# LiangZhaoPKUImperial/LinearSFM

Hardware: AMD Instinct MI355X
Metric: hierarchical linear map-joining solve wall-clock, NC3500-like stereo (all transforms + joins) (lower is better)
Workload: dtype f64

## Files before the change

### linearsfm_amd/csrc/lsfm_small.hip

```cpp
#include "lsfm_device.hpp"
#include "lsfm_internal.hpp"
#include "lsfm_solve.hpp"

namespace lsfm {

#define SM_PASS 16
#define SM_K (3 * SM_PASS)
#define SM_KS (SM_K + 1)
#define SM_THREADS 256
#define SM_CHUNK 256
#define SM_SUPER 64
#define SM_WROWS 1024

typedef double sm_v4d __attribute__((ext_vector_type(4)));

struct SmallArgs {
	int nseg;
	const int *pose_off, *feat_off, *u_off;
	const unsigned char* seg_active;
	const double* U; const int *Ui, *Uj;
	const double* W; const int *photo, *fptr;
	const double* V;
	const double *ea, *eb, *x0;
	const unsigned char* fixed;
	double *x_pose, *x_feat;
	RunStatsDev* run;
	int* status;
	double* max_rel;
	int dbg;
};

template <int NTR>
struct SmallShared {
	static constexpr int R = 16 * NTR;
	double S[R * (R + 1)];
	double P[R * SM_KS];
	double d0[R];
	double E[R], x[R], r[R], v[R], dinv[R];
	double ly[SM_SUPER * 9];
	double wst[SM_WROWS * 3];
	int sph[SM_WROWS / 6 + 1];
	int fpc[2][SM_CHUNK + 1];
	unsigned char fx[R];
	int bad;
	int strips[4];
};

template <int NTR>
#ifndef LSFM_SMALL_OCC
#define LSFM_SMALL_OCC 2
#endif
__global__ void __launch_bounds__(SM_THREADS, NTR >= 6 ? 1 : (NTR <= 2 ? LSFM_SMALL_OCC : 2))
k_small_solve(SmallArgs a)
{
	constexpr int R = 16 * NTR, LD = R + 1;
	constexpr int NTILE = NTR * (NTR + 1) / 2, NW = SM_THREADS / 64, T = (NTILE + NW - 1) / NW;
	extern __shared__ double sm_raw[];
	SmallShared<NTR>& sh = *reinterpret_cast<SmallShared<NTR>*>(sm_raw);
	const int g = blockIdx.x, tid = threadIdx.x, lane = tid & 63, wave = __builtin_amdgcn_readfirstlane(tid >> 6);
	const int p0 = a.pose_off[g], m = a.pose_off[g + 1] - p0, n = 6 * m;
	const int f0 = a.feat_off[g], f1 = a.feat_off[g + 1];
	if (a.seg_active && !a.seg_active[g])
	{
		for (int i = tid; i < n; i += SM_THREADS) a.x_pose[(size_t)p0 * 6 + i] = a.x0 ? a.x0[(size_t)p0 * 6 + i] : 0.0;
		return;
	}
	for (int i = tid; i < R * LD; i += SM_THREADS) sh.S[i] = 0.0;
	for (int i = tid; i < R; i += SM_THREADS)
	{
		sh.E[i] = i < n ? a.ea[(size_t)p0 * 6 + i] : 0.0;
		sh.fx[i] = (i >= n || (a.fixed && a.fixed[(size_t)p0 * 6 + i])) ? 1 : 0;
	}
	if (tid == 0) sh.bad = 0;
	__syncthreads();
	{
		const int u0 = a.u_off[g], u1 = a.u_off[g + 1];
		for (int q = tid; q < (u1 - u0) * 36; q += SM_THREADS)
		{
			const int i = u0 + q / 36, e = q % 36, r = e / 6, c = e % 6;
			const int pa = a.Ui[i] - p0, pb = a.Uj[i] - p0;
			const double v = a.U[(size_t)i * 36 + e];
			lds_add_f64(&sh.S[(6 * pa + r) * LD + 6 * pb + c], v);
			if (pa != pb) lds_add_f64(&sh.S[(6 * pb + c) * LD + 6 * pa + r], v);
		}
	}
	int ti[T], tj[T];
	sm_v4d acc[T];
#pragma unroll
	for (int t = 0; t < T; t++)
	{
		const int q = wave + NW * t;
		int i = 0, j = 0;
		if (q < NTILE)
		{
			while ((j + 1) * (j + 2) / 2 <= q) j++;
			i = q - j * (j + 1) / 2;
		}
		ti[t] = q < NTILE ? i : -1; tj[t] = j;
		acc[t] = (sm_v4d){ 0.0, 0.0, 0.0, 0.0 };
	}
	constexpr int NE = (NTR + NW - 1) / NW;
	double eacc[NE];
#pragma unroll
	for (int i = 0; i < NE; i++) eacc[i] = 0.0;
	const int lbase = (lane & 15) * SM_KS + (lane >> 4);
	constexpr int PF = SM_WROWS / SM_THREADS;
	constexpr int MCAP = R / 6;
	double pw[PF][3];
	int pk[PF];
	double pv[9], pe[3];
	int qbn = 0, c0 = f0, cb = 1;
	auto prefetch = [&](int q0) {
		const int nf = min(SM_SUPER, f1 - q0);
		if (q0 - c0 >= SM_CHUNK || q0 == f0)
		{
			c0 = q0; cb ^= 1;
			for (int i = tid; i <= min(SM_CHUNK, f1 - c0); i += SM_THREADS) sh.fpc[cb][i] = a.fptr[c0 + i];
			__syncthreads();
		}
		qbn = sh.fpc[cb][q0 - c0];
		const int rw = (sh.fpc[cb][q0 - c0 + nf] - qbn) * 6;
		if (tid < nf)
		{
			ld<9>(pv, a.V + (size_t)(q0 + tid) * 9);
			ld<3>(pe, a.eb + (size_t)(q0 + tid) * 3);
		}
		const double* wb = a.W + (size_t)qbn * 18;
#pragma unroll
		for (int i = 0; i < PF; i++)
		{
			const int w = tid + SM_THREADS * i;
			if (w < rw) { pw[i][0] = wb[3 * (size_t)w]; pw[i][1] = wb[3 * (size_t)w + 1]; pw[i][2] = wb[3 * (size_t)w + 2]; pk[i] = a.photo[qbn + w / 6]; }
		}
	};
	for (int i = tid; i < R * SM_KS; i += SM_THREADS) sh.P[i] = 0.0;
	if (f0 < f1) prefetch(f0);
	for (int s0 = f0; s0 < f1; s0 += SM_SUPER)
	{
		const int nfs = min(SM_SUPER, f1 - s0);
		const int qbs = qbn, cs = c0, bs = cb;
		const int rws = (sh.fpc[bs][s0 - cs + nfs] - qbs) * 6;
		__syncthreads();
#pragma unroll
		for (int i = 0; i < PF; i++)
		{
			const int w = tid + SM_THREADS * i;
			if (w < rws)
			{
				sh.wst[3 * w] = pw[i][0]; sh.wst[3 * w + 1] = pw[i][1]; sh.wst[3 * w + 2] = pw[i][2];
				if (w % 6 == 0) sh.sph[w / 6] = pk[i] - p0;
			}
		}
		if (tid < 4) sh.strips[tid] = 0;
		if (tid < SM_SUPER)
		{
			double l[9];
#pragma unroll
			for (int i = 0; i < 9; i++) l[i] = 0.0;
			if (tid < nfs && !(a.dbg & 1))
			{
				double o[9];
				inv3_sym(pv, o);
				const double d0 = o[0];
				l[0] = sqrt(d0); l[1] = o[3] / l[0]; l[3] = o[6] / l[0];
				const double d1 = o[4] - l[1] * l[1];
				l[2] = sqrt(d1); l[4] = (o[7] - l[3] * l[1]) / l[2];
				const double d2 = o[8] - l[3] * l[3] - l[4] * l[4];
				l[5] = sqrt(d2);
				l[6] = l[0] * pe[0] + l[1] * pe[1] + l[3] * pe[2];
				l[7] = l[2] * pe[1] + l[4] * pe[2];
				l[8] = l[5] * pe[2];
				if (!(d0 > 0.0) || !(d1 > 0.0) || !(d2 > 0.0)) sh.bad = 1;
			}
			st<9>(&sh.ly[tid * 9], l);
		}
		__syncthreads();
		if (s0 + SM_SUPER < f1) prefetch(s0 + SM_SUPER);
		for (int sub = 0; sub * SM_PASS < nfs; sub++)
		{
			const int q0 = s0 + sub * SM_PASS, nf = min(SM_PASS, f1 - q0);
			{
				const int lp = tid >> 4, fl = tid & 15;
				bool found = false;
				if (lp < MCAP && !(a.dbg & 2))
				{
					double c18[18];
#pragma unroll
					for (int i = 0; i < 18; i++) c18[i] = 0.0;
					if (fl < nf && lp < m)
					{
						const int j0 = sh.fpc[bs][q0 - cs + fl], j1 = sh.fpc[bs][q0 - cs + fl + 1];
						const double* l = &sh.ly[(sub * SM_PASS + fl) * 9];
						const double l0 = l[0], l1 = l[1], l2 = l[2], l3 = l[3], l4 = l[4], l5 = l[5];
						for (int j = j0; j < j1; j++)
						{
							const int e = j - qbs;
							const int ph = 6 * e < SM_WROWS ? sh.sph[e] : a.photo[j] - p0;
							if (ph != lp) continue;
							found = true;
#pragma unroll
							for (int r = 0; r < 6; r++)
							{
								double w0, w1, w2;
								if (6 * e + 5 < SM_WROWS) { w0 = sh.wst[3 * (6 * e + r)]; w1 = sh.wst[3 * (6 * e + r) + 1]; w2 = sh.wst[3 * (6 * e + r) + 2]; }
								else { const double* wg = a.W + (size_t)j * 18 + 3 * r; w0 = wg[0]; w1 = wg[1]; w2 = wg[2]; }
								c18[3 * r] += w0 * l0 + w1 * l1 + w2 * l3;
								c18[3 * r + 1] += w1 * l2 + w2 * l4;
								c18[3 * r + 2] += w2 * l5;
							}
						}
					}
#pragma unroll
					for (int r = 0; r < 6; r++)
					{
						double* d = &sh.P[(6 * lp + r) * SM_KS + 3 * fl];
						d[0] = c18[3 * r]; d[1] = c18[3 * r + 1]; d[2] = c18[3 * r + 2];
					}
				}
				const int b0 = (6 * lp) >> 4, b1 = (6 * lp + 5) >> 4;
#pragma unroll
				for (int sidx = 0; sidx < NTR; sidx++)
					if (__ballot(found && (b0 == sidx || b1 == sidx)) != 0ull && lane == 0) atomicOr(&sh.strips[sub], 1 << sidx);
			}
			__syncthreads();
			const int smask = sh.strips[sub];
			{
				const int kq = lane >> 4;
#pragma unroll
				for (int si = 0; si < NE; si++)
				{
					const int strip = wave + NW * si;
					if (strip < NTR && ((smask >> strip) & 1) && !(a.dbg & 4))
					{
						const double* pr = &sh.P[(16 * strip + (lane & 15)) * SM_KS + 12 * kq];
						const double* yq = &sh.ly[sub * SM_PASS * 9 + kq * 36 + 6];
						double e0 = 0.0, e1 = 0.0;
#pragma unroll
						for (int k = 0; k < 12; k += 2)
						{
							e0 = fma(pr[k], yq[(k / 3) * 9 + k % 3], e0);
							e1 = fma(pr[k + 1], yq[((k + 1) / 3) * 9 + (k + 1) % 3], e1);
						}
						double sum = e0 + e1;
						sum += __shfl_xor(sum, 16, 64);
						sum += __shfl_xor(sum, 32, 64);
						eacc[si] -= sum;
					}
				}
			}
			bool on[T];
#pragma unroll
			for (int t = 0; t < T; t++) on[t] = ti[t] >= 0 && (((smask >> ti[t]) & (smask >> tj[t]) & 1) != 0) && !(a.dbg & 8);
#pragma unroll 2
			for (int ks = 0; ks < SM_K / 4; ks++)
			{
#pragma unroll
				for (int t = 0; t < T; t++)
				{
					if (!on[t]) continue;
					const double av = sh.P[16 * ti[t] * SM_KS + lbase + 4 * ks], bv = sh.P[16 * tj[t] * SM_KS + lbase + 4 * ks];
					acc[t] = __builtin_amdgcn_mfma_f64_16x16x4f64(av, bv, acc[t], 0, 0, 0);
				}
			}
			__syncthreads();
		}
	}
	__syncthreads();
#pragma unroll
	for (int t = 0; t < T; t++)
	{
		if (ti[t] < 0) continue;
		const int C = 16 * tj[t] + (lane & 15);
#pragma unroll
		for (int e = 0; e < 4; e++)
		{
			const int Rr = 16 * ti[t] + (lane >> 4) + 4 * e;
			const double v = acc[t][e];
			sh.S[Rr * LD + C] -= v;
			if (ti[t] != tj[t]) sh.S[C * LD + Rr] -= v;
		}
	}
	if (lane < 16)
#pragma unroll
		for (int si = 0; si < NE; si++)
		{
			const int strip = wave + NW * si;
			if (strip < NTR) sh.E[16 * strip + lane] += eacc[si];
		}
	__syncthreads();
	for (int q = tid; q < R * R; q += SM_THREADS)
	{
		const int i = q / R, j = q - i * R;
		if (sh.fx[i] || sh.fx[j]) sh.S[i * LD + j] = i == j ? 1.0 : 0.0;
	}
	for (int i = tid; i < R; i += SM_THREADS) if (sh.fx[i]) sh.E[i] = 0.0;
	__syncthreads();
	for (int i = tid; i < R; i += SM_THREADS) sh.d0[i] = sh.S[i * LD + i];
	__syncthreads();
	int pivot_bad = -1;
	for (int j = 0; j < ((a.dbg & 16) ? 0 : n); j++)
	{
		const double d = sh.S[j * LD + j];
		if (!(d > 0.0) || !(d < 1e300)) { pivot_bad = j; break; }
		const double piv = sqrt(d), ip = 1.0 / piv;
		__syncthreads();
		for (int i = j + tid; i < n; i += SM_THREADS) sh.S[i * LD + j] = i == j ? piv : sh.S[i * LD + j] * ip;
		__syncthreads();
		{
			const int ty = tid >> 4, tx = tid & 15;
			for (int i = j + 1 + ty; i < n; i += 16)
			{
				const double lij = sh.S[i * LD + j];
				for (int k = j + 1 + tx; k <= i; k += 16) sh.S[i * LD + k] = fma(-lij, sh.S[k * LD + j], sh.S[i * LD + k]);
			}
		}
		__syncthreads();
	}
	if (pivot_bad >= 0)
	{
		if (tid == 0) { atomicCAS(&a.status[1], 0, 1 + g); if (a.run && !a.run->chol_err) a.run->chol_err = 1 + p0 + pivot_bad / 6; }
		return;
	}
	for (int i = tid; i < n; i += SM_THREADS) sh.dinv[i] = 1.0 / sh.S[i * LD + i];
	__syncthreads();
	auto solve = [&](const double* rhs, double* out) {
		for (int i = tid; i < R; i += SM_THREADS) sh.v[i] = i < n ? rhs[i] : 0.0;
		__syncthreads();
		if (wave == 0)
		{
			for (int j = 0; j < n; j++)
			{
				const double vj = sh.v[j] * sh.dinv[j];
				__builtin_amdgcn_wave_barrier();
				if (lane == 0) sh.v[j] = vj;
				for (int i = j + 1 + lane; i < n; i += 64) sh.v[i] = fma(-sh.S[i * LD + j], vj, sh.v[i]);
				__builtin_amdgcn_wave_barrier();
			}
			for (int j = n - 1; j >= 0; j--)
			{
				const double vj = sh.v[j] * sh.dinv[j];
				__builtin_amdgcn_wave_barrier();
				if (lane == 0) sh.v[j] = vj;
				for (int i = lane; i < j; i += 64) sh.v[i] = fma(-sh.S[j * LD + i], vj, sh.v[i]);
				__builtin_amdgcn_wave_barrier();
			}
		}
		__syncthreads();
		for (int i = tid; i < R; i += SM_THREADS) out[i] = sh.v[i];
		__syncthreads();
	};
	auto residual = [&](const double* xx) {
		for (int i = tid; i < n; i += SM_THREADS)
		{
			double s = sh.E[i] - sh.d0[i] * xx[i];
			for (int j = 0; j < n; j++)
				if (j != i) s = fma(-(i < j ? sh.S[i * LD + j] : sh.S[j * LD + i]), xx[j], s);
			sh.r[i] = s;
		}
		__syncthreads();
	};
	if (!(a.dbg & 16))
	{
	solve(sh.E, sh.x);
	residual(sh.x);
	solve(sh.r, sh.v);
	for (int i = tid; i < n; i += SM_THREADS) sh.x[i] += sh.v[i];
	__syncthreads();
	residual(sh.x);
	}
	if (tid == 0)
	{
		double rr = 0.0, ee = 0.0;
		for (int i = 0; i < n; i++) { rr += sh.r[i] * sh.r[i]; ee += sh.E[i] * sh.E[i]; }
		const double rel = ee > 0.0 ? sqrt(rr / ee) : 0.0;
		if (!(rel < 1e-8) || sh.bad)
		{
			atomicAdd(&a.status[0], 1);
			if (a.run) atomicAdd(&a.run->not_converged, 1);
		}
		const unsigned long long bits = (unsigned long long)__double_as_longlong(rel == rel ? rel : 1e300);
		atomicMax(reinterpret_cast<unsigned long long*>(a.max_rel), bits);
		if (a.run) atomicMax(reinterpret_cast<unsigned long long*>(&a.run->max_rel_residual), bits);
	}
	for (int i = tid; i < n; i += SM_THREADS) a.x_pose[(size_t)p0 * 6 + i] = sh.fx[i] ? 0.0 : sh.x[i];
	for (int f = f0 + tid; f < ((a.dbg & 32) ? f0 : f1); f += SM_THREADS)
	{
		double V[9], iv[9];
		ld<9>(V, a.V + (size_t)f * 9);
		inv3_sym(V, iv);
		double d[3] = { a.eb[(size_t)f * 3], a.eb[(size_t)f * 3 + 1], a.eb[(size_t)f * 3 + 2] };
		double s3[3] = { 0.0, 0.0, 0.0 };
		for (int j = a.fptr[f]; j < a.fptr[f + 1]; j++)
		{
			double w[18];
			ld<18>(w, a.W + (size_t)j * 18);
			const double* xp = &sh.x[6 * (a.photo[j] - p0)];
#pragma unroll
			for (int c = 0; c < 3; c++)
			{
				double sacc = 0.0;
#pragma unroll
				for (int r = 0; r < 6; r++) sacc = fma(w[3 * r + c], sh.fx[6 * (a.photo[j] - p0) + r] ? 0.0 : xp[r], sacc);
				s3[c] += sacc;
			}
		}
		d[0] -= s3[0]; d[1] -= s3[1]; d[2] -= s3[2];
		for (int r = 0; r < 3; r++) a.x_feat[(size_t)f * 3 + r] = iv[3 * r] * d[0] + iv[3 * r + 1] * d[1] + iv[3 * r + 2] * d[2];
	}
}

static int small_solve_strips(int most_poses, int cap)
{
	if (most_poses > cap) return 0;
	if (most_poses <= 2) return 1;
	if (most_poses <= 5) return 2;
	if (most_poses <= 8) return 3;
	if (most_poses <= 16) return 6;
	return 0;
}
int small_level_strips(const lsfm_context* ctx, int most_rows)
{
	return (ctx->small_max > 0 && !ctx->comm && !ctx->pcg.mixed) ? small_solve_strips(most_rows, ctx->small_max) : 0;
}
void small_level_offsets(lsfm_context* ctx, const DevBatch& out, SolveIO& io)
{
	if (!small_level_strips(ctx, io.seg_rows)) return;
	const int G = io.nseg;
	int* d_uo = ctx->scratch.alloc<int>(G + 1);
	h2d(ctx, d_uo, out.u_off.data(), sizeof(int) * (size_t)(G + 1));
	io.d_pose_off = out.d_pose_off; io.d_feat_off = out.d_feat_off; io.d_u_off = d_uo;
}

template <int NTR>
static void launch_small(hipStream_t s, const SmallArgs& a)
{
	const size_t lds = sizeof(SmallShared<NTR>);
	static const bool set = []() {
		(void)hipFuncSetAttribute(reinterpret_cast<const void*>(&k_small_solve<NTR>), hipFuncAttributeMaxDynamicSharedMemorySize, (int)sizeof(SmallShared<NTR>));
		return true;
	}();
	(void)set;
	hipLaunchKernelGGL(k_small_solve<NTR>, dim3(a.nseg), dim3(SM_THREADS), lds, s, a);
}

void small_solve_launch(lsfm_context* ctx, const SolveIO& io, int strips, int* status, double* max_rel)
{
	SmallArgs a;
	a.nseg = io.nseg; a.pose_off = io.d_pose_off; a.feat_off = io.d_feat_off; a.u_off = io.d_u_off; a.seg_active = io.d_seg_active;
	a.U = io.U; a.Ui = io.Ui; a.Uj = io.Uj; a.W = io.W; a.photo = io.photo; a.fptr = io.fptr; a.V = io.V;
	a.ea = io.ea; a.eb = io.eb; a.x0 = io.x0; a.fixed = io.d_fixed; a.x_pose = io.x_pose; a.x_feat = io.x_feat;
	a.run = (ctx->in_tree_run && ctx->d_run) ? ctx->d_run : nullptr;
	a.status = status; a.max_rel = max_rel;
	a.dbg = getenv("LSFM_SMALL_DEBUG") ? atoi(getenv("LSFM_SMALL_DEBUG")) : 0;
	if (!io.nseg) return;
	switch (strips)
	{
	case 1: launch_small<1>(ctx->stream, a); break;
	case 2: launch_small<2>(ctx->stream, a); break;
	case 3: launch_small<3>(ctx->stream, a); break;
	default: launch_small<6>(ctx->stream, a); break;
	}
	LSFM_CHECK_HIP(hipGetLastError());
}

}
```

Baseline: 31.18.

## Give each wave its own feature panel in small Schur kernels to drop block barriers

For the one- and two-tile variants of the small-segment Schur solve, each wave now owns a private P panel and its own slice of the feature super-block. It accumulates all tiles itself and synchronises only at wavefront level instead of with block-wide __syncthreads. Per-wave results are merged into S and E serially, one wave per turn. Photo matching in staging now builds a 32-entry bitmask and iterates its set bits. This is meant to remove block-barrier stalls and idle waves when there are few tiles, at the cost of more LDS for panels and a serialized reduction.

```diff
diff --git a/linearsfm_amd/csrc/lsfm_small.hip b/linearsfm_amd/csrc/lsfm_small.hip
--- a/linearsfm_amd/csrc/lsfm_small.hip
+++ b/linearsfm_amd/csrc/lsfm_small.hip
@@ -5,8 +5,6 @@
 namespace lsfm {
 
 #define SM_PASS 16
-#define SM_K (3 * SM_PASS)
-#define SM_KS (SM_K + 1)
 #define SM_THREADS 256
 #define SM_CHUNK 256
 #define SM_SUPER 64
@@ -31,10 +29,18 @@
 };
 
 template <int NTR>
+struct SmallScheme {
+	static constexpr int WP = NTR == 1 ? 16 : (NTR == 2 ? 8 : 0);
+	static constexpr int PASS = WP ? WP : SM_PASS;
+	static constexpr int KS = 3 * PASS + 1;
+	static constexpr int NPANEL = WP ? SM_THREADS / 64 : 1;
+};
+
+template <int NTR>
 struct SmallShared {
 	static constexpr int R = 16 * NTR;
 	double S[R * (R + 1)];
-	double P[R * SM_KS];
+	double P[SmallScheme<NTR>::NPANEL * R * SmallScheme<NTR>::KS];
 	double d0[R];
 	double E[R], x[R], r[R], v[R], dinv[R];
 	double ly[SM_SUPER * 9];
@@ -45,6 +51,86 @@
 	int bad;
 	int strips[4];
 };
+static_assert(sizeof(SmallShared<1>) <= 80 * 1024 && sizeof(SmallShared<2>) <= 80 * 1024, "k_small_solve<1>, <2>: two work-groups a CU");
+
+template <int KS>
+__device__ __forceinline__ bool sm_stage_cell(const SmallArgs& a, const double* wst, const int* sph, const double* l, bool live, int j0, int j1,
+                                              int qbs, int p0, int lp, double* d)
+{
+	bool found = false;
+	double c18[18];
+#pragma unroll
+	for (int i = 0; i < 18; i++) c18[i] = 0.0;
+	if (live)
+	{
+		const double l0 = l[0], l1 = l[1], l2 = l[2], l3 = l[3], l4 = l[4], l5 = l[5];
+		for (int jb = j0; jb < j1; jb += 32)
+		{
+			unsigned mk = 0;
+			const int je = min(j1, jb + 32);
+#pragma unroll 4
+			for (int j = jb; j < je; j++)
+				mk |= ((6 * (j - qbs) < SM_WROWS ? sph[j - qbs] : a.photo[j] - p0) == lp ? 1u : 0u) << (j - jb);
+			for (; mk; mk &= mk - 1)
+			{
+				const int j = jb + __builtin_ctz(mk);
+				const int e = j - qbs;
+				found = true;
+#pragma unroll
+				for (int r = 0; r < 6; r++)
+				{
+					double w0, w1, w2;
+					if (6 * e + 5 < SM_WROWS) { w0 = wst[3 * (6 * e + r)]; w1 = wst[3 * (6 * e + r) + 1]; w2 = wst[3 * (6 * e + r) + 2]; }
+					else { const double* wg = a.W + (size_t)j * 18 + 3 * r; w0 = wg[0]; w1 = wg[1]; w2 = wg[2]; }
+					c18[3 * r] += w0 * l0 + w1 * l1 + w2 * l3;
+					c18[3 * r + 1] += w1 * l2 + w2 * l4;
+					c18[3 * r + 2] += w2 * l5;
+				}
+			}
+		}
+	}
+#pragma unroll
+	for (int r = 0; r < 6; r++)
+	{
+		d[r * KS] = c18[3 * r]; d[r * KS + 1] = c18[3 * r + 1]; d[r * KS + 2] = c18[3 * r + 2];
+	}
+	return found;
+}
+
+template <int KS>
+__device__ __forceinline__ double sm_strip_py(const double* prow, const double* ly, int kq)
+{
+	constexpr int KQ = (KS - 1) / 4;
+	const double* pr = prow + KQ * kq;
+	const double* yq = ly + kq * (KQ / 3) * 9 + 6;
+	double e0 = 0.0, e1 = 0.0;
+#pragma unroll
+	for (int k = 0; k < KQ; k += 2)
+	{
+		e0 = fma(pr[k], yq[(k / 3) * 9 + k % 3], e0);
+		if (k + 1 < KQ) e1 = fma(pr[k + 1], yq[((k + 1) / 3) * 9 + (k + 1) % 3], e1);
+	}
+	double sum = e0 + e1;
+	sum += __shfl_xor(sum, 16, 64);
+	sum += __shfl_xor(sum, 32, 64);
+	return sum;
+}
+
+template <int KS, int NT, int UNROLL>
+__device__ __forceinline__ void sm_tiles_ppt(const double* pl, const int (&ti)[NT], const int (&tj)[NT], const bool (&on)[NT], sm_v4d (&acc)[NT])
+{
+#pragma unroll UNROLL
+	for (int ks = 0; ks < (KS - 1) / 4; ks++)
+	{
+#pragma unroll
+		for (int t = 0; t < NT; t++)
+		{
+			if (!on[t]) continue;
+			const double av = pl[16 * ti[t] * KS + 4 * ks], bv = pl[16 * tj[t] * KS + 4 * ks];
+			acc[t] = __builtin_amdgcn_mfma_f64_16x16x4f64(av, bv, acc[t], 0, 0, 0);
+		}
+	}
+}
 
 template <int NTR>
 #ifndef LSFM_SMALL_OCC
@@ -54,7 +140,8 @@
 k_small_solve(SmallArgs a)
 {
 	constexpr int R = 16 * NTR, LD = R + 1;
-	constexpr int NTILE = NTR * (NTR + 1) / 2, NW = SM_THREADS / 64, T = (NTILE + NW - 1) / NW;
+	constexpr int WP = SmallScheme<NTR>::WP, PASS = SmallScheme<NTR>::PASS, KS = SmallScheme<NTR>::KS;
+	constexpr int NTILE = NTR * (NTR + 1) / 2, NW = SM_THREADS / 64, T = WP ? NTILE : (NTILE + NW - 1) / NW;
 	extern __shared__ double sm_raw[];
 	SmallShared<NTR>& sh = *reinterpret_cast<SmallShared<NTR>*>(sm_raw);
 	const int g = blockIdx.x, tid = threadIdx.x, lane = tid & 63, wave = __builtin_amdgcn_readfirstlane(tid >> 6);
@@ -89,7 +176,7 @@
 #pragma unroll
 	for (int t = 0; t < T; t++)
 	{
-		const int q = wave + NW * t;
+		const int q = WP ? t : wave + NW * t;
 		int i = 0, j = 0;
 		if (q < NTILE)
 		{
@@ -99,11 +186,11 @@
 		ti[t] = q < NTILE ? i : -1; tj[t] = j;
 		acc[t] = (sm_v4d){ 0.0, 0.0, 0.0, 0.0 };
 	}
-	constexpr int NE = (NTR + NW - 1) / NW;
+	constexpr int NE = WP ? NTR : (NTR + NW - 1) / NW;
 	double eacc[NE];
 #pragma unroll
 	for (int i = 0; i < NE; i++) eacc[i] = 0.0;
-	const int lbase = (lane & 15) * SM_KS + (lane >> 4);
+	const int lbase = (lane & 15) * KS + (lane >> 4);
 	constexpr int PF = SM_WROWS / SM_THREADS;
 	constexpr int MCAP = R / 6;
 	double pw[PF][3];
@@ -133,7 +220,7 @@
 			if (w < rw) { pw[i][0] = wb[3 * (size_t)w]; pw[i][1] = wb[3 * (size_t)w + 1]; pw[i][2] = wb[3 * (size_t)w + 2]; pk[i] = a.photo[qbn + w / 6]; }
 		}
 	};
-	for (int i = tid; i < R * SM_KS; i += SM_THREADS) sh.P[i] = 0.0;
+	for (int i = tid; i < SmallScheme<NTR>::NPANEL * R * KS; i += SM_THREADS) sh.P[i] = 0.0;
 	if (f0 < f1) prefetch(f0);
 	for (int s0 = f0; s0 < f1; s0 += SM_SUPER)
 	{
@@ -151,7 +238,7 @@
 				if (w % 6 == 0) sh.sph[w / 6] = pk[i] - p0;
 			}
 		}
-		if (tid < 4) sh.strips[tid] = 0;
+		if (!WP && tid < 4) sh.strips[tid] = 0;
 		if (tid < SM_SUPER)
 		{
 			double l[9];
@@ -176,118 +263,80 @@
 		}
 		__syncthreads();
 		if (s0 + SM_SUPER < f1) prefetch(s0 + SM_SUPER);
-		for (int sub = 0; sub * SM_PASS < nfs; sub++)
-		{
-			const int q0 = s0 + sub * SM_PASS, nf = min(SM_PASS, f1 - q0);
-			{
-				const int lp = tid >> 4, fl = tid & 15;
+		double* const P = WP ? sh.P + wave * (R * KS) : sh.P;
+		const int id = WP ? lane : tid;
+		constexpr int NL = WP ? 64 : SM_THREADS;
+		auto meet = [&]() {
+			if constexpr (WP != 0) { __builtin_amdgcn_fence(__ATOMIC_ACQ_REL, "wavefront"); __builtin_amdgcn_wave_barrier(); }
+			else __syncthreads();
+		};
+		const int lf_begin = WP ? SM_PASS * wave : 0, lf_end = min(nfs, WP ? SM_PASS * wave + SM_PASS : SM_SUPER);
+		for (int lf0 = lf_begin; lf0 < lf_end; lf0 += PASS)
+		{
+			const int q0 = s0 + lf0, nf = min(PASS, f1 - q0);
+			unsigned seen = 0;
+#pragma unroll
+			for (int c0l = 0; c0l < MCAP * PASS; c0l += NL)
+			{
+				const int c = c0l + id, lp = c / PASS, fl = c % PASS;
 				bool found = false;
 				if (lp < MCAP && !(a.dbg & 2))
 				{
-					double c18[18];
-#pragma unroll
-					for (int i = 0; i < 18; i++) c18[i] = 0.0;
-					if (fl < nf && lp < m)
-					{
-						const int j0 = sh.fpc[bs][q0 - cs + fl], j1 = sh.fpc[bs][q0 - cs + fl + 1];
-						const double* l = &sh.ly[(sub * SM_PASS + fl) * 9];
-						const double l0 = l[0], l1 = l[1], l2 = l[2], l3 = l[3], l4 = l[4], l5 = l[5];
-						for (int j = j0; j < j1; j++)
-						{
-							const int e = j - qbs;
-							const int ph = 6 * e < SM_WROWS ? sh.sph[e] : a.photo[j] - p0;
-							if (ph != lp) continue;
-							found = true;
-#pragma unroll
-							for (int r = 0; r < 6; r++)
-							{
-								double w0, w1, w2;
-								if (6 * e + 5 < SM_WROWS) { w0 = sh.wst[3 * (6 * e + r)]; w1 = sh.wst[3 * (6 * e + r) + 1]; w2 = sh.wst[3 * (6 * e + r) + 2]; }
-								else { const double* wg = a.W + (size_t)j * 18 + 3 * r; w0 = wg[0]; w1 = wg[1]; w2 = wg[2]; }
-								c18[3 * r] += w0 * l0 + w1 * l1 + w2 * l3;
-								c18[3 * r + 1] += w1 * l2 + w2 * l4;
-								c18[3 * r + 2] += w2 * l5;
-							}
-						}
-					}
-#pragma unroll
-					for (int r = 0; r < 6; r++)
-					{
-						double* d = &sh.P[(6 * lp + r) * SM_KS + 3 * fl];
-						d[0] = c18[3 * r]; d[1] = c18[3 * r + 1]; d[2] = c18[3 * r + 2];
-					}
+					const bool live = fl < nf && lp < m;
+					const int j0 = live ? sh.fpc[bs][q0 - cs + fl] : 0, j1 = live ? sh.fpc[bs][q0 - cs + fl + 1] : 0;
+					found = sm_stage_cell<KS>(a, sh.wst, sh.sph, &sh.ly[(lf0 + fl) * 9], live, j0, j1, qbs, p0, lp, &P[6 * lp * KS + 3 * fl]);
 				}
 				const int b0 = (6 * lp) >> 4, b1 = (6 * lp + 5) >> 4;
 #pragma unroll
 				for (int sidx = 0; sidx < NTR; sidx++)
-					if (__ballot(found && (b0 == sidx || b1 == sidx)) != 0ull && lane == 0) atomicOr(&sh.strips[sub], 1 << sidx);
-			}
-			__syncthreads();
-			const int smask = sh.strips[sub];
-			{
-				const int kq = lane >> 4;
+					if (__ballot(found && (b0 == sidx || b1 == sidx)) != 0ull) seen |= 1u << sidx;
+			}
+			if (!WP && lane == 0 && seen) atomicOr(&sh.strips[lf0 / SM_PASS], (int)seen);
+			meet();
+			const int smask = WP ? (int)seen : sh.strips[lf0 / SM_PASS];
+#pragma unroll
+			for (int si = 0; si < NE; si++)
+			{
+				const int strip = WP ? si : wave + NW * si;
+				if (strip < NTR && ((smask >> strip) & 1) && !(a.dbg & 4))
+					eacc[si] -= sm_strip_py<KS>(&P[(16 * strip + (lane & 15)) * KS], &sh.ly[lf0 * 9], lane >> 4);
+			}
+			bool on[T];
+#pragma unroll
+			for (int t = 0; t < T; t++) on[t] = ti[t] >= 0 && (((smask >> ti[t]) & (smask >> tj[t]) & 1) != 0) && !(a.dbg & 8);
+			sm_tiles_ppt<KS, T, (WP ? (KS - 1) / 4 : 2)>(P + lbase, ti, tj, on, acc);
+			meet();
+		}
+	}
+	__syncthreads();
+	for (int turn = 0; turn < (WP ? NW : 1); turn++)
+	{
+		if (!WP || wave == turn)
+		{
+#pragma unroll
+			for (int t = 0; t < T; t++)
+			{
+				if (ti[t] < 0) continue;
+				const int C = 16 * tj[t] + (lane & 15);
+#pragma unroll
+				for (int e = 0; e < 4; e++)
+				{
+					const int Rr = 16 * ti[t] + (lane >> 4) + 4 * e;
+					const double v = acc[t][e];
+					sh.S[Rr * LD + C] -= v;
+					if (ti[t] != tj[t]) sh.S[C * LD + Rr] -= v;
+				}
+			}
+			if (lane < 16)
 #pragma unroll
 				for (int si = 0; si < NE; si++)
 				{
-					const int strip = wave + NW * si;
-					if (strip < NTR && ((smask >> strip) & 1) && !(a.dbg & 4))
-					{
-						const double* pr = &sh.P[(16 * strip + (lane & 15)) * SM_KS + 12 * kq];
-						const double* yq = &sh.ly[sub * SM_PASS * 9 + kq * 36 + 6];
-						double e0 = 0.0, e1 = 0.0;
-#pragma unroll
-						for (int k = 0; k < 12; k += 2)
-						{
-							e0 = fma(pr[k], yq[(k / 3) * 9 + k % 3], e0);
-							e1 = fma(pr[k + 1], yq[((k + 1) / 3) * 9 + (k + 1) % 3], e1);
-						}
-						double sum = e0 + e1;
-						sum += __shfl_xor(sum, 16, 64);
-						sum += __shfl_xor(sum, 32, 64);
-						eacc[si] -= sum;
-					}
+					const int strip = WP ? si : wave + NW * si;
+					if (strip < NTR) sh.E[16 * strip + lane] += eacc[si];
 				}
-			}
-			bool on[T];
-#pragma unroll
-			for (int t = 0; t < T; t++) on[t] = ti[t] >= 0 && (((smask >> ti[t]) & (smask >> tj[t]) & 1) != 0) && !(a.dbg & 8);
-#pragma unroll 2
-			for (int ks = 0; ks < SM_K / 4; ks++)
-			{
-#pragma unroll
-				for (int t = 0; t < T; t++)
-				{
-					if (!on[t]) continue;
-					const double av = sh.P[16 * ti[t] * SM_KS + lbase + 4 * ks], bv = sh.P[16 * tj[t] * SM_KS + lbase + 4 * ks];
-					acc[t] = __builtin_amdgcn_mfma_f64_16x16x4f64(av, bv, acc[t], 0, 0, 0);
-				}
-			}
-			__syncthreads();
-		}
-	}
-	__syncthreads();
-#pragma unroll
-	for (int t = 0; t < T; t++)
-	{
-		if (ti[t] < 0) continue;
-		const int C = 16 * tj[t] + (lane & 15);
-#pragma unroll
-		for (int e = 0; e < 4; e++)
-		{
-			const int Rr = 16 * ti[t] + (lane >> 4) + 4 * e;
-			const double v = acc[t][e];
-			sh.S[Rr * LD + C] -= v;
-			if (ti[t] != tj[t]) sh.S[C * LD + Rr] -= v;
-		}
-	}
-	if (lane < 16)
-#pragma unroll
-		for (int si = 0; si < NE; si++)
-		{
-			const int strip = wave + NW * si;
-			if (strip < NTR) sh.E[16 * strip + lane] += eacc[si];
-		}
-	__syncthreads();
+		}
+		__syncthreads();
+	}
 	for (int q = tid; q < R * R; q += SM_THREADS)
 	{
 		const int i = q / R, j = q - i * R;
```

Result: no change. 31.30, median of 2 (+0.4%).
